# max-andr/joint-cnn-mrf

Measured on AMD Instinct MI355X. Metric: images/sec (720x480, K=9 joints) part-detector+spatial-model fwd, higher is better.
Workload: dtype f32(fp16x2 spectra, fft); 1 GPU; configs[1]: batch=64/GPU synthetic 480x720x3, part detector + spatial model forward + argmax, fp32; batch_per_gpu=64, global_batch=64, micro_batch=64, use_sm=True, collective=all_gather coords int32 [B,2,9]

## Files before the change

### joint-cnn-mrf_amd/csrc/conv_fft.hip

```cpp
#include <cmath>
#include <cstdlib>
#include <map>
#include <mutex>
#include <utility>
#include <vector>

#include "conv_fft_common.h"

namespace jcm {
namespace cfft {

template <int KS, int NP>
__global__ __launch_bounds__(256) void weight_spectra_split_kernel(const float* __restrict__ w, uint4* __restrict__ Ws, int Cin, int Cout, int CoutP, int ntl, int NY, int NX,
                                                                   int round_bf16, float* __restrict__ wscale) {
  __shared__ cf twy[192][KS - 1], twx[KS];
  const int tid = threadIdx.x;
  const int kx = blockIdx.y;
#pragma unroll 1
  for (int k = tid; k < NY * (KS - 1) + KS; k += 256) {
    const bool isy = k < NY * (KS - 1);
    const int ky = k / (KS - 1), a = isy ? k % (KS - 1) + 1 : k - NY * (KS - 1);
    const int num = isy ? (ky * a) % NY : (kx * a) % NX, den = isy ? NY : NX;
    double sn, cs;
    sincospi(-2.0 * (double)num / (double)den, &sn, &cs);
// ... 129 lines not shown
    if (v == n) return off;
    off += v;
  }
  return -1;
}
static bool sizes_of(int H, int W, int ks, Sizes* s, int circ = 0) {
  if (circ) {
    s->NY = H; s->NX = W;
    return (ks == 9 || ks == 5) && H > 8 && W > 8 && tw_offset(H) >= 0 && tw_offset(W) >= 0;
  }
  return (ks == 9 || ks == 5) && H + ks - 1 <= 192 && W + ks - 1 <= 192 && pick(H + 4, &s->NY) && pick(W + 4, &s->NX);
}
static int pad64(int c) { return (c + CB - 1) / CB * CB; }
static bool fft_reg_on() {
  static const bool on = [] { const char* e = std::getenv("JCM_FFT_REG"); return !e || std::atoi(e) != 0; }();
  return on;
}
static int padn(int c, int n) { return (c + n - 1) / n * n; }

int persistent_grid(const void* kernel, int ntiles, int threads, int dyn_lds) {
  static std::mutex mu;
  static std::map<std::pair<const void*, int>, int> cache;
  int dev = 0;
  (void)hipGetDevice(&dev);
  int resident = 0;
  {
    std::lock_guard<std::mutex> lk(mu);
    auto it = cache.find({kernel, dev});
    if (it != cache.end()) resident = it->second;
  }
// ... 76 lines not shown
  p.F = s.NY * p.NXH;
  p.ldy = padn(a.Cout, cgemm_split_ntile(np, a.Cout));
  if (p.ldy < pad64(a.Cout)) p.ldy = pad64(a.Cout);
  p.MT = cgemm_split_mtile(np, a.B, a.Cout);
  const size_t cop = pad64(a.Cout), cmax = (size_t)a.Cin > cop ? a.Cin : cop;
  const size_t bp = (size_t)(a.B + p.MT - 1) / p.MT * p.MT;
  p.t_bytes = (size_t)a.B * p.NXH * a.H * cmax * sizeof(cf);
  p.xs_bytes = (size_t)p.F * bp * a.Cin * 4 * cgemm_split_parts(np);
  p.yf_bytes = (size_t)p.F * a.B * p.ldy * sizeof(cf);
  p.inv_cb = s.NY > 100 ? 32 : 64;
  p.sc_fwd_bytes = (size_t)a.B * a.H * (a.Cin / CB) * sizeof(float);
  p.sc_inv_bytes = (size_t)a.B * p.NXH * (cop / p.inv_cb) * sizeof(float);
  return p;
}
size_t align256(size_t v) { return (v + 255) & ~size_t(255); }
}
size_t conv_fft_workspace_bytes(const ConvArgs& a, int ks, int np) {
  Sizes s;
  if (!sizes_of(a.H, a.W, ks, &s, a.circ)) return 0;
  const Plan3 p = plan_of(a, s, np);
  return align256(p.t_bytes) + align256(p.xs_bytes) + align256(p.yf_bytes) + align256(p.sc_fwd_bytes) + align256(p.sc_inv_bytes);
}
bool conv_fft_fusable(const ConvArgs& a, int ks, int ks_next) {
  Sizes s, n;
  return sizes_of(a.H, a.W, ks, &s) && sizes_of(a.H, a.W, ks_next, &n) && s.NX == n.NX && a.Cout % CB == 0;
}
size_t conv_fft_handover_bytes(const ConvArgs& a, int ks) {
  Sizes s;
  if (!sizes_of(a.H, a.W, ks, &s)) return 0;
  return (size_t)a.B * (s.NX / 2 + 1) * a.H * a.Cout * sizeof(cf);
}
bool conv_fft_win_gather_supported(int win, int Cin) { return fft_reg_on() && cfft_rows_fwd_win_reg_supported(win, Cin); }
bool conv_fft_win_scatter_supported(int win, int Cout) { return fft_reg_on() && win == 32 && Cout % 64 == 0; }
bool conv_fft_pool_fusable(const ConvArgs& a, int ks, int ks_next) {
  Sizes s, n;
  return sizes_of(a.H, a.W, ks, &s) && sizes_of((a.H + 1) / 2, (a.W + 1) / 2, ks_next, &n) && cfft_rows_inv_pool_fwd_supported(s.NX, n.NX, a.Cout);
}
size_t conv_fft_pool_handover_bytes(const ConvArgs& a, int ks_next) {
  Sizes n;
  if (!sizes_of((a.H + 1) / 2, (a.W + 1) / 2, ks_next, &n)) return 0;
  return (size_t)a.B * (n.NX / 2 + 1) * ((a.H + 1) / 2) * a.Cout * sizeof(cf);
}
bool conv_fft_merge_fusable(const ConvArgs& a, int ks, int ks_next, const FftMerge& m, bool h16) {
  Sizes s;
  if (!conv_fft_fusable(a, ks, ks_next) || !sizes_of(a.H, a.W, ks, &s)) return false;
  const bool reg = fft_reg_on() && cfft_rows_inv_merge_fwd_reg_supported(s.NX, a, m, (ks - 1) / 2);
  return h16 ? reg : (reg || cfft_rows_inv_merge_fwd_supported(s.NX, a, m));
}
hipError_t conv_fft_f32(const ConvArgs& a0, int ks, int np, int in_layout, int out_layout, void* work, const void* t_in, void* t_next, const FftMerge* merge,
                        hipEvent_t g0, hipEvent_t g1, hipStream_t st, void* xs, bool xs_ready, const Fp16Scale* scp, const FftNext* nx) {
  Sizes s;
  if (!conv_fft_supported(a0, ks) || !sizes_of(a0.H, a0.W, ks, &s, a0.circ) || (out_layout == 2 && a0.Cout % 8) || (np != 2 && np != 4 && np != 5) || (np == 5 && a0.Cin % 32)) return hipErrorInvalidValue;
  if (a0.circ && (t_in || t_next || merge || in_layout != 0 || out_layout != 0)) return hipErrorInvalidValue;
  if (nx && (nx->pool || nx->merge) && (!t_next || (nx->pool && nx->merge))) return hipErrorInvalidValue;
  Fp16Scale sc;
  if (np >= 4) {
    if (!scp || !scp->tmax || !scp->winv || (t_next && !scp->tmax_next)) return hipErrorInvalidValue;
    sc = *scp;
    sc.hf = (float)a0.H;
    sc.nb = a0.B;
  }
  const bool h16 = sc.t16 && ((t_next && nx && nx->merge && !t_in) || (t_in && !t_next));
  if ((t_in || t_next) && !h16 && (in_layout != 0 || out_layout != 0)) return hipErrorInvalidValue;
  if (t_next && a0.Cout % CB) return hipErrorInvalidValue;
  if (sc.t16 && (np != 5 || in_layout == 0 || out_layout == 0 || xs || ((t_in || t_next) && !h16))) return hipErrorInvalidValue;
// ... 96 lines not shown
```

### joint-cnn-mrf_amd/csrc/conv_fft_common.h

```cpp
#pragma once
#include "fft_lds.h"
#include "kernels.h"

namespace jcm {
namespace cfft {
using namespace fftl;
constexpr int CB = 64, NT = 256;
constexpr int kParMax = 512;

template <int N> struct Plan;
template <> struct Plan<192> { static constexpr int R1 = 8, R2 = 8, R3 = 3; };
template <> struct Plan<128> { static constexpr int R1 = 8, R2 = 4, R3 = 4; };
template <> struct Plan<100> { static constexpr int R1 = 4, R2 = 5, R3 = 5; };
template <> struct Plan<96> { static constexpr int R1 = 8, R2 = 12, R3 = 1; };
template <> struct Plan<72> { static constexpr int R1 = 8, R2 = 3, R3 = 3; };
template <> struct Plan<64> { static constexpr int R1 = 8, R2 = 8, R3 = 1; };
template <> struct Plan<60> { static constexpr int R1 = 4, R2 = 15, R3 = 1; };
template <> struct Plan<50> { static constexpr int R1 = 5, R2 = 10, R3 = 1; };
template <> struct Plan<40> { static constexpr int R1 = 8, R2 = 5, R3 = 1; };
template <> struct Plan<36> { static constexpr int R1 = 4, R2 = 3, R3 = 3; };
template <> struct Plan<32> { static constexpr int R1 = 8, R2 = 4, R3 = 1; };
template <> struct Plan<28> { static constexpr int R1 = 4, R2 = 7, R3 = 1; };
template <> struct Plan<24> { static constexpr int R1 = 8, R2 = 3, R3 = 1; };
template <> struct Plan<20> { static constexpr int R1 = 4, R2 = 5, R3 = 1; };
// ... 230 lines not shown
    default: CALL(192); break;                   \
  }

int persistent_grid(const void* kernel, int ntiles, int threads, int dyn_lds = 0);

void cfft_rows_fwd(int NX, const ConvArgs& a, int layout, cf* T, const cf* tw, float* tmax, hipStream_t st, float* t16 = nullptr);
void cfft_rows_fwd_merge(int NX, const ConvArgs& a, const FftMerge& m, int in_layout, cf* T, const cf* tw, float* tmax, hipStream_t st, float* t16 = nullptr);
hipError_t cfft_cols_fwd(int NY, const ConvArgs& a, int np, const cf* T, void* Xs, const cf* tw, int NXH, int MT, const Fp16Scale& sc, hipStream_t st);
void cfft_cols_inv(int NY, const ConvArgs& a, const cf* Yf, cf* T, const cf* tw, int NXH, int ldy, int pad, hipStream_t st, float* t16 = nullptr, float y16_inv = 0.f);
void cfft_rows_inv(int NX, const ConvArgs& a, int layout, const cf* T, const cf* tw, int pad, float norm, const Fp16Scale& sc, hipStream_t st);
bool cfft_rows_inv_reg(int NX, const ConvArgs& a, int layout, const cf* T, int pad, float norm, const Fp16Scale& sc, hipStream_t st);
bool cfft_rows_inv_fwd_reg(int NX, const ConvArgs& a, const cf* T, cf* Tn, int pad, float norm, const Fp16Scale& sc, hipStream_t st);
bool cfft_rows_fwd_reg(int NX, const ConvArgs& a, int layout, cf* T, float* tmax, hipStream_t st, float* t16);
bool cfft_rows_fwd_win_reg(int NX, const ConvArgs& a, cf* T, float* tmax, hipStream_t st);
bool cfft_rows_fwd_win_reg_supported(int NX, int Cin);
bool cfft_rows_fwd_merge_reg(int NX, const ConvArgs& a, const FftMerge& m, int in_layout, cf* T, float* tmax, hipStream_t st, float* t16);
bool cfft_cols_inv_reg(int NY, const ConvArgs& a, const cf* Yf, cf* T, int NXH, int ldy, int pad, hipStream_t st, float* t16, float y16_inv = 0.f);
void cfft_rows_inv_fwd(int NX, const ConvArgs& a, const cf* T, cf* Tn, const cf* tw, int pad, float norm, const Fp16Scale& sc, hipStream_t st);
bool cfft_rows_inv_pool_fwd(int NXI, int NXO, const ConvArgs& a, const cf* T, cf* Tn, const cf* twi, const cf* two, int pad, float norm, const Fp16Scale& sc, hipStream_t st);
bool cfft_rows_inv_merge_fwd(int NX, const ConvArgs& a, const FftMerge& m, const cf* T, cf* Tn, const cf* tw, int pad, float norm, const Fp16Scale& sc, hipStream_t st);
bool cfft_rows_inv_merge_fwd_reg(int NX, const ConvArgs& a, const FftMerge& m, const cf* T, cf* Tn, int pad, float norm, const Fp16Scale& sc, hipStream_t st, float* t16n = nullptr);
bool cfft_rows_inv_merge_fwd_reg_supported(int NX, const ConvArgs& a, const FftMerge& m, int pad);
bool cfft_rows_inv_pool_fwd_supported(int NXI, int NXO, int Cout);
bool cfft_rows_inv_mfma(int NX, const ConvArgs& a, int layout, const cf* T, int pad, float norm, const Fp16Scale& sc, hipStream_t st);
bool cfft_rows_inv_merge_fwd_supported(int NX, const ConvArgs& a, const FftMerge& m);
}
}
```

### joint-cnn-mrf_amd/csrc/conv_fft_rows_reg.hip

```cpp
#include "conv_fft_common.h"
#include "fft_reg.h"
#include "resize_tf1.h"

namespace jcm {
namespace cfft {
using namespace fftr;

template <int NX, int K1, bool ALL = false, class St>
__device__ __forceinline__ void inv_rows_out2(const cf (&u)[NX / 2], int h, int W, int pad, St&& store) {
  constexpr int M = NX / 2, R1 = RPlan<M>::R1, R2 = RPlan<M>::R2;
  cf o[R2];
  step2_row<M, 1, K1>(u, o);
#pragma unroll
  for (int k2 = 0; k2 < R2; ++k2) {
    const int xo = 2 * (K1 + R1 * k2) + h - pad;
    if (ALL || (xo >= 0 && xo < W)) store(K1 + R1 * k2, xo, o[k2]);
  }
  __builtin_amdgcn_sched_barrier(0);
  if constexpr (K1 + 1 < R1) inv_rows_out2<NX, K1 + 1, ALL>(u, h, W, pad, store);
}
template <int NX, int N>
__device__ __forceinline__ void inv_rows_in2(cf (&u)[NX / 2], const float4& q1, const float4& q2, float sg, bool odd) {
  constexpr int M = NX / 2;
  if constexpr (N == 0) {
// ... 479 lines not shown
  }
  __builtin_amdgcn_sched_barrier(0);
  unsigned raw[M];
  merge_px<NX, W, W3, 0>(raw, r1, v2, v3, odd);
  fwd_rows_finish<NX>(raw, T, h, p, b, y, B, H, C, tmax, t16);
}
bool cfft_rows_fwd_merge_reg(int NX, const ConvArgs& a, const FftMerge& m, int in_layout, cf* T, float* tmax, hipStream_t st, float* t16) {
  if (NX != 96 || in_layout != 1 || !t16 || a.Cin % 64 || a.W != 90 || m.W2 != 45 || m.W3 != 23 || m.H2 < 1 || m.H3 < 1) return false;
  const int nrows = a.B * a.H;
  const size_t threads = a.Cin == 512 ? (size_t)((nrows + 3) / 4) * 8 * 256 : (size_t)nrows * a.Cin;
  hipLaunchKernelGGL((rows_fwd_merge_reg_kernel<96, 90, 23>), dim3((unsigned)((threads + 255) / 256)), dim3(256), 0, st, static_cast<const unsigned*>(a.x), static_cast<const unsigned*>(m.x2), m.H2,
                     static_cast<const unsigned*>(m.x3), m.H3, reinterpret_cast<uint2*>(T), nrows, a.B, a.H, a.Cin, (float)m.H2 / (float)a.H, (float)m.H3 / (float)a.H, tmax, t16);
  return true;
}

template <int NX, int PAD, int I, class Act>
__device__ __forceinline__ void fused_rows_mid(const cf (&x)[NX / 2], cf (&uu)[NX / 2], bool odd, int h, int W, Act&& act) {
  constexpr int M = NX / 2, R1 = RPlan<M>::R1, R2 = RPlan<M>::R2, Q = M / 2;
  constexpr int ma = I + PAD / 2, mb = I + Q + PAD / 2;
  cf a = cf{0.f, 0.f}, bq = cf{0.f, 0.f};
  if constexpr (ma < M) { if (2 * I + h < W) a = act(x[R2 * (ma % R1) + ma / R1]); }
  if constexpr (mb < M) { if (2 * (I + Q) + h < W) bq = act(x[R2 * (mb % R1) + mb / R1]); }
  const cf sm = a + bq, df = a - bq;
  const cf keep = cf{odd ? df.x : sm.x, odd ? df.y : sm.y}, send = cf{odd ? sm.x : df.x, odd ? sm.y : df.y};
  const cf recv = cf{__uint_as_float((unsigned)__builtin_amdgcn_mov_dpp((int)__float_as_uint(send.x), 0xB1, 0xF, 0xF, true)),
                     __uint_as_float((unsigned)__builtin_amdgcn_mov_dpp((int)__float_as_uint(send.y), 0xB1, 0xF, 0xF, true))};
  cf e = cf{odd ? recv.x : keep.x, odd ? recv.y : keep.y}, o = cf{odd ? keep.x : recv.x, odd ? keep.y : recv.y};
  if constexpr (I > 0) {
    const float wr = odd ? Tw<-2 * I, NX>::re : 1.f, wi = odd ? Tw<-2 * I, NX>::im : 0.f;
    e = cf{fmaf(-e.y, wi, e.x * wr), fmaf(e.x, wi, e.y * wr)};
  }
  {
    const float wr = odd ? Tw<-(2 * I + 1), NX>::re : 1.f, wi = odd ? Tw<-(2 * I + 1), NX>::im : 0.f;
    o = cf{fmaf(-o.y, wi, o.x * wr), fmaf(o.x, wi, o.y * wr)};
  }
  uu[2 * I] = e;
  uu[2 * I + 1] = o;
  if constexpr (I + 1 < Q) fused_rows_mid<NX, PAD, I + 1>(x, uu, odd, h, W, act);
}
template <int NX, int PAD>
__global__ __launch_bounds__(256) __attribute__((amdgpu_waves_per_eu(2, 2))) void rows_inv_fwd_reg_kernel(const float4* __restrict__ T, float4* __restrict__ Tn, const float* __restrict__ bias,
                                                                                                  const float* __restrict__ scale, const float* __restrict__ shift, int relu_bn, int nrows,
                                                                                                  int B, int H, int W, int C, float norm0, Fp16Scale sc) {
  constexpr int NXH = NX / 2 + 1, M = NX / 2;
  const int CP = C >> 1;
  const size_t g = (size_t)blockIdx.x * 256 + threadIdx.x;
  const int h = (int)(g & 1), lane = threadIdx.x & 63;
  const int p = (int)((g >> 1) % CP);
  const size_t by = (size_t)(unsigned)__builtin_amdgcn_readfirstlane((int)((g >> 1) / CP));
  if (by >= (size_t)nrows) return;
  const int b = (int)(by / H), y = (int)(by % H), c = 2 * p;
  const bool odd = h != 0;
// ... 287 lines not shown
  else if (layout == 1 && a.Cout % 8 == 0) RR_LAUNCH(1, false);
  else if (layout == 2 && h16 && a.Cout % 8 == 0) RR_LAUNCH(2, true);
  else if (layout == 2 && a.Cout % 8 == 0) RR_LAUNCH(2, false);
  else return false;
#undef RR_LAUNCH
  return true;
}
bool cfft_rows_inv_reg(int NX, const ConvArgs& a, int layout, const cf* T, int pad, float norm, const Fp16Scale& sc, hipStream_t st) {
  if (NX == 96) return launch_rows_inv_reg<96>(a, layout, T, pad, norm, sc, st);
  if (NX == 32 && layout == 0) return launch_rows_inv_reg<32>(a, layout, T, pad, norm, sc, st);
  if (NX == 50) return launch_rows_inv_reg<50>(a, layout, T, pad, norm, sc, st);
  if (NX == 28) return launch_rows_inv_reg<28>(a, layout, T, pad, norm, sc, st);
  return false;
}

}
}
```

### joint-cnn-mrf_amd/csrc/ctx.h

```cpp
#pragma once
#include "../../include/jcm.h"

#include <map>
#include <mutex>
#include <string>
#include <vector>

#include "kernels.h"

namespace jcm {

struct CallOrder;

int fail(int code, const std::string& msg);

#define HIP_TRY(expr)                                                                                   \
  do {                                                                                                  \
    hipError_t e_ = (expr);                                                                             \
    if (e_ != hipSuccess)                                                                               \
      return ::jcm::fail(JCM_ERR_HIP, std::string(#expr) + ": " + hipGetErrorString(e_));               \
  } while (0)
#define JCM_TRY(expr)          \
  do {                         \
    int r_ = (expr);           \
// ... 63 lines not shown
  float* sp_energy = nullptr;
  float* sp_bias = nullptr;
  float* bn_sm_scale = nullptr;
  float* bn_sm_shift = nullptr;
  int* cond = nullptr;
  const float** energy_ptrs = nullptr;
  const float** bias_ptrs = nullptr;
  int* cond0 = nullptr;
  int sm_algo = 3;
  void* fft_t_next = nullptr;
  const void* fft_t_in = nullptr;
  void* fft_xs = nullptr;
  bool fft_xs_ready = false;
  void* sm_scratch = nullptr;
  unsigned sm_epoch = 0;
  int fft_fuse = 3;
  int bf16_hpool = 1;
  int conv_hpool = 0;
  int fft_rows_mfma = 1;
  int fft_next_pool = 0, fft_next_ks = 0;
  const void* fft_win_map = nullptr;
  int fft_win_B = 0, fft_win_H = 0, fft_win_W = 0, fft_win_TY = 0, fft_win_TX = 0;
  bool fft_win_scatter = false;
  bool fft_t_in_16 = false;
  const void* fft_next_merge = nullptr;
  const void* fft_merge = nullptr;
  int conv9_fft = 1;
  int fft_single = 1;
  int fft_win = 1;
  int fft_t16 = 1;
// ... 100 lines not shown
```

### joint-cnn-mrf_amd/csrc/jcm_api.hip

```cpp
#include <cmath>
#include <cstdlib>
#include <cstdio>
#include <cstring>

#include <mutex>
#include <vector>

#include "ctx.h"

using namespace jcm;

namespace {
thread_local std::string g_err;
}

namespace jcm {

const char* const kJointNames[10] = {"lsho", "lelb", "lwri", "rsho", "relb", "rwri", "lhip", "rhip", "nose", "torso"};

int fail(int code, const std::string& msg) {
  g_err = msg;
  return code;
}

// ... 235 lines not shown
    if (hipError_t e = hipMemsetAsync(b.p, 0, (size_t)b.cap * sizeof(float), c->stream); e != hipSuccess) {
      (void)hipFree(b.p);
      return fail(JCM_ERR_HIP, std::string("hipMemsetAsync: ") + hipGetErrorString(e));
    }
    c->fft_blocks.push_back(b);
  }
}
int run_conv_fft(jcm_ctx* c, const ConvLayer* L, const std::string& scope, const void* x, int B, int H, int W, void* out, int in_layout, int out_layout, int circ) {
  ConvArgs a{};
  a.x = x; a.bias = L->bias; a.scale = L->scale; a.shift = L->shift; a.out = out;
  a.B = B; a.H = H; a.W = W; a.Cin = L->cin; a.Cout = L->cout; a.CoutP = L->cout; a.relu_bn = L->has_bn ? 1 : 0;
  a.circ = circ;
  a.rows_mfma = c->fft_rows_mfma;
  const size_t mark = c->arena_off;
  const int np = fft_np(c);
  void* work = arena_alloc<char>(c, conv_fft_workspace_bytes(a, L->ks, np));
  c->arena_off = mark;
  if (c->dry) { c->fft_t_in = nullptr; c->fft_t_next = nullptr; c->fft_merge = nullptr; c->fft_xs = nullptr; c->fft_xs_ready = false; c->fft_tmax_in = nullptr; c->fft_next_pool = 0; c->fft_next_ks = 0; c->fft_next_merge = nullptr; c->fft_t_in_16 = false; c->fft_win_map = nullptr; c->fft_win_scatter = false; return JCM_OK; }
  const std::string key = scope + (circ ? "@win" : "@") + std::to_string(H) + "x" + std::to_string(W);
  if (!c->fft_w.count(key)) {
    static const size_t cap = [] { const char* e = std::getenv("JCM_FFT_CACHE_GB"); return (size_t)(e ? std::atoi(e) : 64) << 30; }();
    const size_t need = conv_fft_weight_bytes(H, W, L->ks, L->cin, L->cout, np, circ);
    size_t held = 0;
    for (auto& kv : c->fft_w) held += kv.second.bytes;
    if (held + need > cap && !c->fft_w.empty()) {
      HIP_TRY(hipStreamSynchronize(c->stream));
      for (auto& kv : c->fft_w) (void)hipFree(kv.second.p);
      c->fft_w.clear();
    }
  }
  jcm_ctx::FftW& fw = c->fft_w[key];
  if (!fw.p) {
    const size_t wb = (conv_fft_weight_bytes(H, W, L->ks, L->cin, L->cout, np, circ) + 255) & ~size_t(255);
    fw.bytes = wb + 256;
    if (hipMalloc(&fw.p, fw.bytes) == hipSuccess) {
      fw.wscale = reinterpret_cast<float*>(static_cast<char*>(fw.p) + wb);
    } else {
      const size_t mb = fw.bytes >> 20;
      c->fft_w.erase(key);
      return fail(JCM_ERR_HIP, "out of device memory for the filter spectra of '" + scope + "' (" + std::to_string(mb) + " MB); jcm_set_option(\"conv9_fft\", 0) selects the direct kernels");
    }
  }
  if (!fw.valid) {
    const float* bound_from = nullptr;
    if (np >= 4 && scope.compare(0, 6, "dgrad:") == 0) {
      auto it = c->fft_w.find(key.substr(6));
      if (it != c->fft_w.end() && it->second.valid && it->second.wscale) bound_from = it->second.wscale;
    }
    HIP_TRY(conv_fft_pack_weights(L->w_raw, fw.p, H, W, L->ks, L->cin, L->cout, np, c->precision == JCM_PRECISION_BF16, c->stream, fw.wscale, circ, bound_from));
    fw.valid = true;
  }
  a.wp = fw.p;
  hipEvent_t e0 = nullptr, e1 = nullptr, g0 = nullptr, g1 = nullptr;
  JCM_TRY(prof_begin(c, &e0, &e1));
  if (c->profile && (pool_get(c, &g0) != JCM_OK || pool_get(c, &g1) != JCM_OK)) { g0 = g1 = nullptr; }
  const void* t_in = c->fft_t_in;
  void* t_next = c->fft_t_next;
  const FftMerge* mg = static_cast<const FftMerge*>(c->fft_merge);
  void* xs = c->fft_xs;
  const bool xs_ready = c->fft_xs_ready;
  FftNext nx;
  nx.pool = c->fft_next_pool; nx.ks_next = c->fft_next_ks; nx.merge = static_cast<const FftMerge*>(c->fft_next_merge);
  c->fft_next_pool = 0; c->fft_next_ks = 0; c->fft_next_merge = nullptr;
  const bool t_in_16 = c->fft_t_in_16;
  c->fft_t_in_16 = false;
  if (c->fft_win_map) {
    a.win_map = c->fft_win_map; a.win_B = c->fft_win_B; a.win_H = c->fft_win_H; a.win_W = c->fft_win_W; a.win_TY = c->fft_win_TY; a.win_TX = c->fft_win_TX;
    c->fft_win_map = nullptr;
  }
  if (c->fft_win_scatter) {
    a.wout_H = c->fft_win_H; a.wout_W = c->fft_win_W; a.wout_TY = c->fft_win_TY; a.wout_TX = c->fft_win_TX;
    c->fft_win_scatter = false;
  }
  Fp16Scale sc;
  if (np >= 4) {
    sc.tmax = c->fft_tmax_in;
    if ((t_in || xs_ready) && !sc.tmax) return fail(JCM_ERR_STATE, "conv_fft '" + scope + "': a handed-over tensor without its scale word");
    if (!sc.tmax) JCM_TRY(fft_new_words(c, B, &sc.tmax));
    if (t_next) JCM_TRY(fft_new_words(c, B, &sc.tmax_next));
    sc.winv = fw.wscale + 1;
    sc.common = c->train ? 1 : 0;
    sc.t16 = (np == 5 && c->fft_t16 && in_layout != 0 && out_layout != 0 && !xs && (!t_in || t_in_16) && (!t_next || (nx.merge && !t_in))) ? 1 : 0;
  }
  c->fft_t_in = nullptr; c->fft_t_next = nullptr; c->fft_merge = nullptr; c->fft_xs = nullptr; c->fft_xs_ready = false;
  c->fft_tmax_in = sc.tmax_next;
  c->fft_last_tmax = sc.tmax;
  const hipError_t e = conv_fft_f32(a, L->ks, np, in_layout, out_layout, work, t_in, t_next, mg, g0, g1, c->stream, xs, xs_ready, np >= 4 ? &sc : nullptr, &nx);
  if (g0 && g1 && e == hipSuccess) c->prof[scope + "/gemm"].emplace_back(g0, g1);
  else { if (g0) c->event_pool.push_back(g0); if (g1) c->event_pool.push_back(g1); }
  prof_end(c, scope, e0, e1, e == hipSuccess);
  if (e != hipSuccess) return fail(JCM_ERR_HIP, std::string("conv_fft_f32: ") + hipGetErrorString(e));
  return JCM_OK;
}
// ... 419 lines not shown
    if ((value != 0) != (h->fft_single != 0)) {
      HIP_TRY(hipStreamSynchronize(h->stream));
      for (auto& kv : h->fft_w) (void)hipFree(kv.second.p);
      h->fft_w.clear();
    }
    h->fft_single = value != 0;
    return JCM_OK;
  }
  if (k == "fft_windows") {
    h->fft_win = value != 0;
    return JCM_OK;
  }
  if (k == "fft_fuse") {
    if (value < 0 || value > 3) return fail(JCM_ERR_ARG, "fft_fuse must be 0..3 (bit 0: pool hand-over, bit 1: merge hand-over)");
    h->fft_fuse = (int)value;
    return JCM_OK;
  }
  if (k == "bf16_hpool") {
    h->bf16_hpool = value != 0;
    return JCM_OK;
  }
  if (k == "fft_rows_mfma") {
    h->fft_rows_mfma = value != 0;
    return JCM_OK;
  }
  if (k == "fft_t16") {
    h->fft_t16 = value != 0;
    return JCM_OK;
  }
  if (k == "sm_chunk") {
// ... 408 lines not shown
```

### joint-cnn-mrf_amd/csrc/kernels.h

```cpp
#pragma once
#include <hip/hip_runtime.h>
#include <stdint.h>

#include <atomic>

namespace jcm {

struct LdsAttr {
  std::atomic<uint64_t> done{0};
  hipError_t ensure(const void* fn, int bytes) {
    int dev = 0;
    hipError_t e = hipGetDevice(&dev);
    if (e != hipSuccess) return e;
    const uint64_t bit = 1ull << (dev & 63);
    if (done.load(std::memory_order_acquire) & bit) return hipSuccess;
    e = hipFuncSetAttribute(fn, hipFuncAttributeMaxDynamicSharedMemorySize, bytes);
    if (e == hipSuccess) done.fetch_or(bit, std::memory_order_release);
    return e;
  }
};

struct ConvArgs {
  const void* x;
  const void* wp;
  const float* bias;
  const float* scale;
  const float* shift;
  void* out;
  int B, H, W, Cin, Cout, CoutP;
  int relu_bn;
  const float* in_scale = nullptr;
  const float* w_scale = nullptr;
  int in_planar = 0, out_planar = 0;
  int circ = 0;
  const void* win_map = nullptr;
  int win_B = 0, win_H = 0, win_W = 0, win_TY = 0, win_TX = 0, win_valid_only = 0;
  int wout_H = 0, wout_W = 0, wout_TY = 0, wout_TX = 0;
  int rows_mfma = 0;
  int hpool = 0;
};
int conv_igemm_bn(int Cout);
hipError_t conv_igemm_f32(const ConvArgs& a, int ks, hipStream_t st);
hipError_t pack_weights_f32(const float* w_hwio, float* wp, int ks, int Cin, int Cout, int CoutP, hipStream_t st);

bool conv_split_supported(int ks, int Cin, int CoutP, int B, int H, int W, int min_wgs);
size_t conv_split_weight_bytes(int ks, int Cin, int CoutP, int ns);
hipError_t pack_weights_split(const float* w_hwio, void* wp, int ks, int Cin, int Cout, int CoutP, int ns, hipStream_t st,
                              const float* w_scale = nullptr);
hipError_t conv_split_f32(const ConvArgs& a, int ks, int ns, hipStream_t st);

hipError_t conv_thin_split16(const ConvArgs& a, hipStream_t st);

// ... 14 lines not shown
  int t16_cb = 64;
};
bool conv_fft_supported(const ConvArgs& a, int ks);
size_t conv_fft_weight_bytes(int H, int W, int ks, int Cin, int Cout, int np, int circ = 0);
hipError_t conv_fft_pack_weights(const float* w_hwio, void* wf, int H, int W, int ks, int Cin, int Cout, int np, bool round_bf16, hipStream_t st,
                                 float* wscale = nullptr, int circ = 0,
                                 const float* bound_from = nullptr);
size_t conv_fft_workspace_bytes(const ConvArgs& a, int ks, int np);
struct FftMerge { const void* x2; int H2, W2; const void* x3; int H3, W3; };
struct FftNext { int pool = 0; int ks_next = 0; const FftMerge* merge = nullptr; };
hipError_t conv_fft_f32(const ConvArgs& a, int ks, int np, int in_layout, int out_layout, void* work, const void* t_in, void* t_next, const FftMerge* merge,
                        hipEvent_t g0, hipEvent_t g1, hipStream_t st, void* xs = nullptr, bool xs_ready = false, const Fp16Scale* sc = nullptr, const FftNext* nx = nullptr);
bool conv_fft_win_gather_supported(int win, int Cin);
bool conv_fft_win_scatter_supported(int win, int Cout);
bool conv_fft_pool_fusable(const ConvArgs& a, int ks, int ks_next);
size_t conv_fft_pool_handover_bytes(const ConvArgs& a, int ks_next);
bool conv_fft_merge_fusable(const ConvArgs& a, int ks, int ks_next, const FftMerge& m, bool h16 = false);
size_t conv_fft_xs_bytes(const ConvArgs& a, int ks, int np);
hipError_t conv_fft_spectra(const ConvArgs& a, int ks, int np, void* work, void* xs, hipStream_t st, float* tmax = nullptr, int common = 0);
bool conv_fft_geometry(int H, int W, int ks, int B, int Cout, int np, int* NY, int* NX, int* MT, int circ = 0);

size_t wgrad_fft_scratch_bytes(int NY, int NX, int Cin, int Cout);
hipError_t wgrad_fft(const void* xs, const void* zs, void* scratch, const float* w, float lmbd, float* dw, int ks, int NY, int NX, int B, int MTx, int MTz, int Cin,
                     int ldz, int Cout, hipStream_t st, int np = 3, const float* tmax_x = nullptr, const float* tmax_z = nullptr, int H = 0);
hipError_t pad_channels_f32(const float* in, int ldi, float* out, int ldo, size_t N, hipStream_t st);
hipError_t window_gather_f32(const float* map, float* win, int B, int H, int W, int C, int WS, int TY, int TX, int valid_only, hipStream_t st);
hipError_t window_scatter_f32(const float* val, float* map, int B, int H, int W, int C, int WS, int TY, int TX, hipStream_t st);
bool conv_fft_fusable(const ConvArgs& a, int ks, int ks_next);
size_t conv_fft_handover_bytes(const ConvArgs& a, int ks);

// ... 147 lines not shown
```

### joint-cnn-mrf_amd/engine.py

```python
import ctypes

import numpy as np
import torch

from . import _lib


def _hm_size(n):
    for _ in range(3):
        n = (n + 1) // 2
    return n


class Engine:

    def __init__(self, device=0, precision='fp32', n_joints=9, stream=None, f32_conv=None, split_min_wgs=None, micro_batch=None, conv9_fft=None, call_order=None, fft_single=None, fft_t16=None, fft_fuse=None):
        if not torch.cuda.is_available():
            raise RuntimeError('joint-cnn-mrf_amd needs an MI355X (gfx950) GPU; torch.cuda.is_available() is False '
                               'and there is no CPU path')
        self._lib = _lib.load()
        self.device = torch.device('cuda', device if isinstance(device, int) else torch.device(device).index or 0)
        self.n_joints = int(n_joints)
        self.precision = precision
        self._stream = stream if stream is not None else torch.cuda.current_stream(self.device)
        h = ctypes.c_void_p()
        _lib.check(self._lib.jcm_create(self.device.index, ctypes.c_void_p(self._stream.cuda_stream), ctypes.byref(h)),
                   'jcm_create')
        self._h = h
        self._finalized = False
        prec = {'fp32': _lib.JCM_PRECISION_F32, 'f32': _lib.JCM_PRECISION_F32, 'bf16': _lib.JCM_PRECISION_BF16}[precision]
        _lib.check(self._lib.jcm_set_option(self._h, b'precision', prec), 'jcm_set_option(precision)')
        _lib.check(self._lib.jcm_set_option(self._h, b'n_joints', self.n_joints), 'jcm_set_option(n_joints)')
        if f32_conv is not None:
            if f32_conv not in ('exact', 'split16'):
                raise ValueError("f32_conv must be 'exact' or 'split16' (the bf16x6 arm 'split' was retired in round 5)")
            _lib.check(self._lib.jcm_set_option(self._h, b'f32_conv', {'exact': 0, 'split16': 2}[f32_conv]), 'jcm_set_option(f32_conv)')
        if micro_batch is not None:
            self.set_micro_batch(micro_batch)
        if conv9_fft is not None:
            self.set_conv9_fft(conv9_fft)
        if fft_single is not None:
            self.set_option('fft_single', int(bool(fft_single)))
        if fft_t16 is not None:
            self.set_option('fft_t16', int(bool(fft_t16)))
        if fft_fuse is not None:
            self.set_option('fft_fuse', int(fft_fuse))
        if call_order is not None:
            self.set_option('call_order', int(bool(call_order)))
        if split_min_wgs is not None:
            _lib.check(self._lib.jcm_set_option(self._h, b'split_min_wgs', int(split_min_wgs)), 'jcm_set_option(split_min_wgs)')

    def close(self):
        if getattr(self, '_h', None) is not None and self._h.value:
            self._lib.jcm_destroy(self._h)
            self._h = ctypes.c_void_p()

    def __del__(self):
        try:
            self.close()
        except Exception:
            pass
# ... 292 lines not shown
```

Measured before the change: 7014 images/sec.

## Split 5x5 FFT convolution into four overlap-save tiles with fused pool hand-over

Adds a tiled FFT convolution path for the 5x5 layer feeding a pooled 5x5 layer: each image is cut into four quadrants with halos, transformed at a smaller FFT size (64x96), convolved per tile, and the inverse row pass stitches the two column tiles, pools and produces the next layer's forward row spectra. The smaller transform size is meant to cut FFT padding overhead and spectrum memory for the full-resolution layer. It adds new row kernels, per-tile scale words and separate weight spectra keyed by the tile size. The cost is halo recomputation and more complex indexing, and the path is restricted to width 180.

```diff
diff --git a/joint-cnn-mrf_amd/csrc/conv_fft.hip b/joint-cnn-mrf_amd/csrc/conv_fft.hip
--- a/joint-cnn-mrf_amd/csrc/conv_fft.hip
+++ b/joint-cnn-mrf_amd/csrc/conv_fft.hip
@@ -167,6 +167,10 @@
 static int pad64(int c) { return (c + CB - 1) / CB * CB; }
 static bool fft_reg_on() {
   static const bool on = [] { const char* e = std::getenv("JCM_FFT_REG"); return !e || std::atoi(e) != 0; }();
+  return on;
+}
+static bool fft_tiles_on() {
+  static const bool on = [] { const char* e = std::getenv("JCM_FFT_TILES"); return !e || std::atoi(e) != 0; }();
   return on;
 }
 static int padn(int c, int n) { return (c + n - 1) / n * n; }
@@ -273,11 +277,17 @@
   return p;
 }
 size_t align256(size_t v) { return (v + 255) & ~size_t(255); }
+ConvArgs tile_view(const ConvArgs& a, const Sizes& s) {
+  ConvArgs t = a;
+  t.B = 4 * a.B; t.H = s.NY; t.W = a.W / 2;
+  t.tiles = 0;
+  return t;
+}
 }
 size_t conv_fft_workspace_bytes(const ConvArgs& a, int ks, int np) {
   Sizes s;
-  if (!sizes_of(a.H, a.W, ks, &s, a.circ)) return 0;
-  const Plan3 p = plan_of(a, s, np);
+  if (!(a.tiles ? sizes_of(a.H / 2, a.W / 2, ks, &s) : sizes_of(a.H, a.W, ks, &s, a.circ))) return 0;
+  const Plan3 p = a.tiles ? plan_of(tile_view(a, s), s, np) : plan_of(a, s, np);
   return align256(p.t_bytes) + align256(p.xs_bytes) + align256(p.yf_bytes) + align256(p.sc_fwd_bytes) + align256(p.sc_inv_bytes);
 }
 bool conv_fft_fusable(const ConvArgs& a, int ks, int ks_next) {
@@ -300,14 +310,53 @@
   if (!sizes_of((a.H + 1) / 2, (a.W + 1) / 2, ks_next, &n)) return 0;
   return (size_t)a.B * (n.NX / 2 + 1) * ((a.H + 1) / 2) * a.Cout * sizeof(cf);
 }
+bool conv_fft_tiles_supported(const ConvArgs& a, int ks, int ks_next) {
+  Sizes s;
+  return fft_reg_on() && fft_tiles_on() && ks == 5 && ks_next == 5 && !a.circ && !a.win_map && a.B >= 1 && conv_fft_pool_fusable(a, ks, ks_next) &&
+         a.H % 4 == 0 && a.W % 4 == 0 && sizes_of(a.H / 2, a.W / 2, ks, &s) && cfft_tiles_supported(s.NY, s.NX, a);
+}
 bool conv_fft_merge_fusable(const ConvArgs& a, int ks, int ks_next, const FftMerge& m, bool h16) {
   Sizes s;
   if (!conv_fft_fusable(a, ks, ks_next) || !sizes_of(a.H, a.W, ks, &s)) return false;
   const bool reg = fft_reg_on() && cfft_rows_inv_merge_fwd_reg_supported(s.NX, a, m, (ks - 1) / 2);
   return h16 ? reg : (reg || cfft_rows_inv_merge_fwd_supported(s.NX, a, m));
 }
+static hipError_t conv_fft_tiles_f32(const ConvArgs& a0, int ks, int np, int in_layout, void* work, const void* t_in, void* t_next, const FftMerge* merge,
+                                     hipEvent_t g0, hipEvent_t g1, hipStream_t st, void* xs, bool xs_ready, const Fp16Scale* scp, const FftNext* nx) {
+  Sizes s;
+  if (np != 4 || in_layout != 0 || t_in || merge || xs || xs_ready || !t_next || !nx || !nx->pool || nx->merge || !scp || !scp->tmax || !scp->winv || !scp->tmax_next ||
+      !conv_fft_tiles_supported(a0, ks, nx->ks_next) || !sizes_of(a0.H / 2, a0.W / 2, ks, &s))
+    return hipErrorInvalidValue;
+  ConvArgs a = a0;
+  a.CoutP = pad64(a.Cout);
+  const ConvArgs at = tile_view(a, s);
+  const Plan3 p = plan_of(at, s, np);
+  Fp16Scale sc = *scp;
+  sc.hf = (float)s.NY;
+  sc.nb = at.B;
+  char* wk = static_cast<char*>(work);
+  cf* T = reinterpret_cast<cf*>(wk);
+  void* Xs = wk + align256(p.t_bytes);
+  cf* Yf = reinterpret_cast<cf*>(wk + align256(p.t_bytes) + align256(p.xs_bytes));
+  int dev = 0;
+  if (hipError_t e = hipGetDevice(&dev); e != hipSuccess) return e;
+  const cf* twb = twiddle_table(dev);
+  if (!twb) return hipErrorOutOfMemory;
+  if (!cfft_rows_fwd_tile_reg(s.NY, s.NX, a, T, sc.tmax, st)) return hipErrorInvalidValue;
+  if (hipError_t ce = cfft_cols_fwd(s.NY, at, np, T, Xs, twb + tw_offset(s.NY), p.NXH, p.MT, sc, st); ce != hipSuccess) return ce;
+  if (hipError_t e = hipGetLastError(); e != hipSuccess) return e;
+  if (g0 && hipEventRecord(g0, st) != hipSuccess) return hipErrorUnknown;
+  if (hipError_t e = cgemm_split(Xs, a.wp, Yf, np, p.F, at.B, a.Cin, a.Cout, p.ldy, st, 0.f); e != hipSuccess) return e;
+  if (g1 && hipEventRecord(g1, st) != hipSuccess) return hipErrorUnknown;
+  ConvArgs ai = at;
+  ai.H = a.H / 2;
+  if (!cfft_cols_inv_reg(s.NY, ai, Yf, T, p.NXH, p.ldy, (ks - 1) / 2, st, nullptr, 0.f)) return hipErrorInvalidValue;
+  if (!cfft_rows_inv_pool_tile_reg(s.NY, s.NX, a, T, static_cast<cf*>(t_next), 1.0f / (float)(s.NY * s.NX), sc, st)) return hipErrorInvalidValue;
+  return hipGetLastError();
+}
 hipError_t conv_fft_f32(const ConvArgs& a0, int ks, int np, int in_layout, int out_layout, void* work, const void* t_in, void* t_next, const FftMerge* merge,
                         hipEvent_t g0, hipEvent_t g1, hipStream_t st, void* xs, bool xs_ready, const Fp16Scale* scp, const FftNext* nx) {
+  if (a0.tiles) return conv_fft_tiles_f32(a0, ks, np, in_layout, work, t_in, t_next, merge, g0, g1, st, xs, xs_ready, scp, nx);
   Sizes s;
   if (!conv_fft_supported(a0, ks) || !sizes_of(a0.H, a0.W, ks, &s, a0.circ) || (out_layout == 2 && a0.Cout % 8) || (np != 2 && np != 4 && np != 5) || (np == 5 && a0.Cin % 32)) return hipErrorInvalidValue;
   if (a0.circ && (t_in || t_next || merge || in_layout != 0 || out_layout != 0)) return hipErrorInvalidValue;
diff --git a/joint-cnn-mrf_amd/csrc/conv_fft_common.h b/joint-cnn-mrf_amd/csrc/conv_fft_common.h
--- a/joint-cnn-mrf_amd/csrc/conv_fft_common.h
+++ b/joint-cnn-mrf_amd/csrc/conv_fft_common.h
@@ -268,6 +268,9 @@
 bool cfft_rows_fwd_reg(int NX, const ConvArgs& a, int layout, cf* T, float* tmax, hipStream_t st, float* t16);
 bool cfft_rows_fwd_win_reg(int NX, const ConvArgs& a, cf* T, float* tmax, hipStream_t st);
 bool cfft_rows_fwd_win_reg_supported(int NX, int Cin);
+bool cfft_tiles_supported(int NY, int NX, const ConvArgs& a);
+bool cfft_rows_fwd_tile_reg(int NY, int NX, const ConvArgs& a, cf* T, float* tmax, hipStream_t st);
+bool cfft_rows_inv_pool_tile_reg(int NY, int NX, const ConvArgs& a, const cf* T, cf* Tn, float norm, const Fp16Scale& sc, hipStream_t st);
 bool cfft_rows_fwd_merge_reg(int NX, const ConvArgs& a, const FftMerge& m, int in_layout, cf* T, float* tmax, hipStream_t st, float* t16);
 bool cfft_cols_inv_reg(int NY, const ConvArgs& a, const cf* Yf, cf* T, int NXH, int ldy, int pad, hipStream_t st, float* t16, float y16_inv = 0.f);
 void cfft_rows_inv_fwd(int NX, const ConvArgs& a, const cf* T, cf* Tn, const cf* tw, int pad, float norm, const Fp16Scale& sc, hipStream_t st);
diff --git a/joint-cnn-mrf_amd/csrc/conv_fft_rows_reg.hip b/joint-cnn-mrf_amd/csrc/conv_fft_rows_reg.hip
--- a/joint-cnn-mrf_amd/csrc/conv_fft_rows_reg.hip
+++ b/joint-cnn-mrf_amd/csrc/conv_fft_rows_reg.hip
@@ -1,3 +1,5 @@
+#include <type_traits>
+
 #include "conv_fft_common.h"
 #include "fft_reg.h"
 #include "resize_tf1.h"
@@ -517,13 +519,8 @@
   return true;
 }
 
-template <int NX, int PAD, int I, class Act>
-__device__ __forceinline__ void fused_rows_mid(const cf (&x)[NX / 2], cf (&uu)[NX / 2], bool odd, int h, int W, Act&& act) {
-  constexpr int M = NX / 2, R1 = RPlan<M>::R1, R2 = RPlan<M>::R2, Q = M / 2;
-  constexpr int ma = I + PAD / 2, mb = I + Q + PAD / 2;
-  cf a = cf{0.f, 0.f}, bq = cf{0.f, 0.f};
-  if constexpr (ma < M) { if (2 * I + h < W) a = act(x[R2 * (ma % R1) + ma / R1]); }
-  if constexpr (mb < M) { if (2 * (I + Q) + h < W) bq = act(x[R2 * (mb % R1) + mb / R1]); }
+template <int NX, int I>
+__device__ __forceinline__ void fwd_rows_mid_pair(const cf a, const cf bq, cf (&uu)[NX / 2], bool odd) {
   const cf sm = a + bq, df = a - bq;
   const cf keep = cf{odd ? df.x : sm.x, odd ? df.y : sm.y}, send = cf{odd ? sm.x : df.x, odd ? sm.y : df.y};
   const cf recv = cf{__uint_as_float((unsigned)__builtin_amdgcn_mov_dpp((int)__float_as_uint(send.x), 0xB1, 0xF, 0xF, true)),
@@ -539,6 +536,15 @@
   }
   uu[2 * I] = e;
   uu[2 * I + 1] = o;
+}
+template <int NX, int PAD, int I, class Act>
+__device__ __forceinline__ void fused_rows_mid(const cf (&x)[NX / 2], cf (&uu)[NX / 2], bool odd, int h, int W, Act&& act) {
+  constexpr int M = NX / 2, R1 = RPlan<M>::R1, R2 = RPlan<M>::R2, Q = M / 2;
+  constexpr int ma = I + PAD / 2, mb = I + Q + PAD / 2;
+  cf a = cf{0.f, 0.f}, bq = cf{0.f, 0.f};
+  if constexpr (ma < M) { if (2 * I + h < W) a = act(x[R2 * (ma % R1) + ma / R1]); }
+  if constexpr (mb < M) { if (2 * (I + Q) + h < W) bq = act(x[R2 * (mb % R1) + mb / R1]); }
+  fwd_rows_mid_pair<NX, I>(a, bq, uu, odd);
   if constexpr (I + 1 < Q) fused_rows_mid<NX, PAD, I + 1>(x, uu, odd, h, W, act);
 }
 template <int NX, int PAD>
@@ -856,5 +862,199 @@
   return false;
 }
 
-}
-}
+
+template <int NX, int J>
+__device__ __forceinline__ void fwd_rows_in2_f32(cf (&u)[NX / 2], const cf (&raw)[NX / 2], float sg, bool odd) {
+  constexpr int M = NX / 2;
+  const cf a = raw[J], o = cf{__uint_as_float(pair_word(__float_as_uint(a.x), odd)), __uint_as_float(pair_word(__float_as_uint(a.y), odd))};
+  cf v = cf{fmaf(sg, a.x, o.x), fmaf(sg, a.y, o.y)};
+  if constexpr (J > 0) {
+    const float wr = odd ? Tw<-J, NX>::re : 1.f, wi = odd ? Tw<-J, NX>::im : 0.f;
+    v = cf{fmaf(-v.y, wi, v.x * wr), fmaf(v.x, wi, v.y * wr)};
+  }
+  u[J] = v;
+  if constexpr (J + 1 < M) fwd_rows_in2_f32<NX, J + 1>(u, raw, sg, odd);
+}
+template <int NX>
+__global__ __launch_bounds__(256) __attribute__((amdgpu_waves_per_eu(3, 3))) void rows_fwd_tile_reg_kernel(const float* __restrict__ map, float4* __restrict__ T, int nrows, int NY,
+                                                                                                   int Hm, int Wm, int Ht, int Wt, int C, float* __restrict__ tmax) {
+  constexpr int M = NX / 2;
+  const int CP = C >> 1;
+  int h, p;
+  size_t by;
+  pair_coords(CP, h, p, by);
+  if (by >= (size_t)nrows) return;
+  const int bt = (int)(by / NY), t = (int)(by % NY);
+  const int tx = bt & 1, ty = (bt >> 1) & 1, b = bt >> 2;
+  const int ym = t < Ht + 2 ? ty * Ht + t : (t >= NY - 2 ? ty * Ht + t - NY : -1);
+  const bool row_in = ym >= 0 && ym < Hm;
+  const auto d = __builtin_amdgcn_make_buffer_rsrc(const_cast<float*>(map) + ((size_t)b * Hm + (row_in ? ym : 0)) * Wm * C, 0, row_in ? Wm * C * 4 : 0, 0x00020000);
+  cf raw[M];
+  typedef float f2 __attribute__((ext_vector_type(2)));
+#pragma unroll
+  for (int j = 0; j < M; ++j) {
+    const int n = h * M + j;
+    const int xm = n < Wt + 2 ? tx * Wt + n : (n >= NX - 2 ? tx * Wt + n - NX : -1);
+    const int off = xm >= 0 && xm < Wm ? xm * C * 4 : Wm * C * 4;
+    raw[j] = __builtin_bit_cast(cf, __builtin_amdgcn_raw_buffer_load_b64(d, p * 8 + off, 0, 0));
+  }
+  const bool odd = h != 0;
+  cf u[M];
+  fwd_rows_in2_f32<NX, 0>(u, raw, odd ? -1.f : 1.f, odd);
+  step1<M, -1>(u);
+  step2_inplace<M, -1, 0>(u);
+  const int cblk = p >> 5, v = p & 31, B4 = nrows / NY;
+  float4* dst = T + ((((size_t)cblk * 4 + (v >> 3)) * B4 + bt) * NY + t) * 8 + (v & 7);
+  const size_t kstride = (size_t)(C >> 4) * B4 * NY * 8;
+  float m = 0.f;
+  fwd_rows_visit<NX, 0>(u, odd, [&](int mi, const float4& o) __attribute__((always_inline)) {
+    const int k = 2 * mi + h;
+    if (k <= M) {
+      dst[(size_t)k * kstride] = o;
+      m = fmaxf(fmaxf(m, fmaxf(fabsf(o.x), fabsf(o.y))), fmaxf(fabsf(o.z), fabsf(o.w)));
+    }
+  });
+  if (tmax) {
+#pragma unroll
+    for (int o = 32; o > 0; o >>= 1) m = fmaxf(m, __shfl_xor(m, o));
+    if ((threadIdx.x & 63) == 0 && m > 0.f) atomicMax(reinterpret_cast<unsigned*>(tmax + bt), __float_as_uint(m));
+  }
+}
+
+template <int NX, int TX, int I, int WT, class Act>
+__device__ __forceinline__ void pool_tile_px(const cf x, cf (&zp)[NX / 2], bool odd, bool first, Act&& act) {
+  const cf v = act(x);
+  const cf w = cf{__uint_as_float((unsigned)__builtin_amdgcn_mov_dpp((int)__float_as_uint(v.x), 0xB1, 0xF, 0xF, true)),
+                  __uint_as_float((unsigned)__builtin_amdgcn_mov_dpp((int)__float_as_uint(v.y), 0xB1, 0xF, 0xF, true))};
+  const cf pm = cf{fmaxf(v.x, w.x), fmaxf(v.y, w.y)};
+  constexpr int q = TX * (WT / 2) + I;
+  if (((q & 1) != 0) == odd) zp[q >> 1] = first ? pm : cf{fmaxf(zp[q >> 1].x, pm.x), fmaxf(zp[q >> 1].y, pm.y)};
+}
+template <int NX, int TX, int K1, int K2, int WT, class Act>
+__device__ __forceinline__ void pool_tile_outs(const cf (&o)[RPlan<NX / 2>::R2], cf (&zp)[NX / 2], bool odd, bool first, Act&& act) {
+  constexpr int I = K1 + RPlan<NX / 2>::R1 * K2 - 1;
+  if constexpr (I >= 0 && I < WT / 2) pool_tile_px<NX, TX, I, WT>(o[K2], zp, odd, first, act);
+  if constexpr (K2 + 1 < RPlan<NX / 2>::R2) pool_tile_outs<NX, TX, K1, K2 + 1, WT>(o, zp, odd, first, act);
+}
+template <int NX, int TX, int K1, int WT, class Act>
+__device__ __forceinline__ void pool_tile_row(const cf (&u)[NX / 2], cf (&zp)[NX / 2], bool odd, bool first, Act&& act) {
+  constexpr int M = NX / 2;
+  cf o[RPlan<M>::R2];
+  step2_row<M, 1, K1>(u, o);
+  pool_tile_outs<NX, TX, K1, 0, WT>(o, zp, odd, first, act);
+  __builtin_amdgcn_sched_barrier(0);
+  if constexpr (K1 + 1 < RPlan<M>::R1) pool_tile_row<NX, TX, K1 + 1, WT>(u, zp, odd, first, act);
+}
+template <int NX, int I>
+__device__ __forceinline__ void pool_rows_mid(const cf (&zp)[NX / 2], cf (&uu)[NX / 2], bool odd) {
+  fwd_rows_mid_pair<NX, I>(zp[I], zp[I + NX / 4], uu, odd);
+  if constexpr (I + 1 < NX / 4) pool_rows_mid<NX, I + 1>(zp, uu, odd);
+}
+template <int NX, int WT>
+__global__ __launch_bounds__(256) __attribute__((amdgpu_waves_per_eu(2, 2))) void rows_inv_pool_tile_reg_kernel(const float4* __restrict__ T, float4* __restrict__ Tn, const float* __restrict__ bias,
+                                                                                                        const float* __restrict__ scale, const float* __restrict__ shift, int relu_bn,
+                                                                                                        int nrows, int B, int Ht, int C, float norm0, Fp16Scale sc) {
+  constexpr int NXH = NX / 2 + 1, M = NX / 2;
+  static_assert(WT % 2 == 0 && WT + 4 <= NX, "even tile width with its halo inside the transform");
+  const int CP = C >> 1;
+  const size_t g = (size_t)blockIdx.x * 256 + threadIdx.x;
+  const int h = (int)(g & 1), lane = threadIdx.x & 63;
+  const int p = (int)((g >> 1) % CP);
+  const size_t by = (size_t)(unsigned)__builtin_amdgcn_readfirstlane((int)((g >> 1) / CP));
+  if (by >= (size_t)nrows) return;
+  const int b = (int)(by / Ht), r = (int)(by % Ht), c = 2 * p;
+  constexpr int KS = (WT / 2 - 1) / 2;
+  __shared__ cf stash[4][KS][64];
+  const int ty = (2 * r) / Ht, yt = 2 * r - ty * Ht;
+  const bool odd = h != 0;
+  const float b0v = bias[c], b1v = bias[c + 1];
+  float s0 = 1.f, s1 = 1.f, h0 = 0.f, h1 = 0.f;
+  if (relu_bn) { s0 = scale[c]; h0 = shift[c]; s1 = scale[c + 1]; h1 = shift[c + 1]; }
+  float tcommon = 0.f;
+  if (sc.tmax && sc.common) {
+    for (int i = lane; i < sc.nb; i += 64) tcommon = fmaxf(tcommon, sc.tmax[i]);
+#pragma unroll
+    for (int o = 32; o > 0; o >>= 1) tcommon = fmaxf(tcommon, __shfl_xor(tcommon, o));
+  }
+  cf zp[M];
+#pragma unroll
+  for (int k = 0; k < M; ++k) zp[k] = cf{0.f, 0.f};
+  auto tile = [&](auto txc) __attribute__((always_inline)) {
+    constexpr int tx = decltype(txc)::value;
+    const int bt = (b * 2 + ty) * 2 + tx;
+    const float norm = sc.tmax ? norm0 * sc.winv[0] * fp16_unscale(sc.common ? tcommon : sc.tmax[bt], sc.hf) : norm0;
+    auto act = [&](cf z) __attribute__((always_inline)) {
+      float v0 = fmaf(z.x, norm, b0v), v1 = fmaf(z.y, norm, b1v);
+      if (relu_bn) { v0 = fmaf(fmaxf(v0, 0.f), s0, h0); v1 = fmaf(fmaxf(v1, 0.f), s1, h1); }
+      return cf{v0, v1};
+    };
+#pragma unroll
+    for (int rr = 0; rr < 2; ++rr) {
+      __builtin_amdgcn_sched_barrier(0);
+      cf u[M];
+      const auto d = __builtin_amdgcn_make_buffer_rsrc(const_cast<float4*>(T) + (((size_t)bt * Ht + yt + rr) * NXH * C) / 2, 0, NXH * C * 8, 0x00020000);
+      const int vo = p * 16, ko = CP * 16;
+      auto load = [&](int k) __attribute__((always_inline)) {
+        typedef float f4 __attribute__((ext_vector_type(4)));
+        const f4 q = __builtin_bit_cast(f4, __builtin_amdgcn_raw_buffer_load_b128(d, vo, k * ko, 0));
+        return make_float4(q[0], q[1], q[2], q[3]);
+      };
+      int hr = h;
+      asm volatile("" : "+v"(hr));
+      const bool odd_r = hr != 0;
+      inv_rows_load2<NX, false, 0>(u, odd_r ? -1.f : 1.f, odd_r, load);
+      step1<M, 1>(u);
+      pool_tile_row<NX, tx, 0, WT>(u, zp, odd, rr == 0, act);
+    }
+  };
+  cf(*const slice)[64] = stash[threadIdx.x >> 6];
+  tile(std::integral_constant<int, 0>{});
+#pragma unroll
+  for (int k = 0; k < KS; ++k) slice[k][lane] = zp[k];
+  tile(std::integral_constant<int, 1>{});
+#pragma unroll
+  for (int k = 0; k < KS; ++k) zp[k] = slice[k][lane];
+  cf uu[M];
+  pool_rows_mid<NX, 0>(zp, uu, odd);
+  step1<M, -1>(uu);
+  step2_inplace<M, -1, 0>(uu);
+  const int cblk = p >> 5, v = p & 31;
+  float4* dst = Tn + ((((size_t)cblk * 4 + (v >> 3)) * B + b) * Ht + r) * 8 + (v & 7);
+  const size_t kstride = (size_t)(C >> 4) * B * Ht * 8;
+  float m = 0.f;
+  fwd_rows_visit<NX, 0>(uu, odd, [&](int mi, const float4& o) __attribute__((always_inline)) {
+    const int k = 2 * mi + h;
+    if (k <= M) {
+      dst[(size_t)k * kstride] = o;
+      m = fmaxf(fmaxf(m, fmaxf(fabsf(o.x), fabsf(o.y))), fmaxf(fabsf(o.z), fabsf(o.w)));
+    }
+  });
+  if (sc.tmax_next) {
+#pragma unroll
+    for (int o = 32; o > 0; o >>= 1) m = fmaxf(m, __shfl_xor(m, o));
+    if (lane == 0 && m > 0.f) atomicMax(reinterpret_cast<unsigned*>(sc.tmax_next + b), __float_as_uint(m));
+  }
+}
+bool cfft_tiles_supported(int NY, int NX, const ConvArgs& a) {
+  return NX == 96 && NY == 64 && a.W == 180 && a.H % 4 == 0 && a.H / 2 + 4 <= NY && a.Cin % 64 == 0 && a.Cout % 64 == 0 &&
+         (size_t)a.W * a.Cin * 4 < (size_t)1 << 31;
+}
+bool cfft_rows_fwd_tile_reg(int NY, int NX, const ConvArgs& a, cf* T, float* tmax, hipStream_t st) {
+  if (!cfft_tiles_supported(NY, NX, a)) return false;
+  const int nrows = 4 * a.B * NY;
+  const size_t threads = (size_t)nrows * a.Cin;
+  hipLaunchKernelGGL(rows_fwd_tile_reg_kernel<96>, dim3((unsigned)((threads + 255) / 256)), dim3(256), 0, st, static_cast<const float*>(a.x), reinterpret_cast<float4*>(T), nrows, NY,
+                     a.H, a.W, a.H / 2, a.W / 2, a.Cin, tmax);
+  return true;
+}
+bool cfft_rows_inv_pool_tile_reg(int NY, int NX, const ConvArgs& a, const cf* T, cf* Tn, float norm, const Fp16Scale& sc, hipStream_t st) {
+  if (!cfft_tiles_supported(NY, NX, a)) return false;
+  const int Ht = a.H / 2, nrows = a.B * Ht;
+  const size_t threads = (size_t)nrows * a.Cout;
+  hipLaunchKernelGGL((rows_inv_pool_tile_reg_kernel<96, 90>), dim3((unsigned)((threads + 255) / 256)), dim3(256), 0, st, reinterpret_cast<const float4*>(T), reinterpret_cast<float4*>(Tn),
+                     a.bias, a.scale, a.shift, a.relu_bn, nrows, a.B, Ht, a.Cout, norm, sc);
+  return true;
+}
+
+}
+}
diff --git a/joint-cnn-mrf_amd/csrc/ctx.h b/joint-cnn-mrf_amd/csrc/ctx.h
--- a/joint-cnn-mrf_amd/csrc/ctx.h
+++ b/joint-cnn-mrf_amd/csrc/ctx.h
@@ -101,6 +101,7 @@
   bool fft_xs_ready = false;
   void* sm_scratch = nullptr;
   unsigned sm_epoch = 0;
+  int fft_tiles = 1;
   int fft_fuse = 3;
   int bf16_hpool = 1;
   int conv_hpool = 0;
diff --git a/joint-cnn-mrf_amd/csrc/jcm_api.hip b/joint-cnn-mrf_amd/csrc/jcm_api.hip
--- a/joint-cnn-mrf_amd/csrc/jcm_api.hip
+++ b/joint-cnn-mrf_amd/csrc/jcm_api.hip
@@ -273,13 +273,16 @@
   a.rows_mfma = c->fft_rows_mfma;
   const size_t mark = c->arena_off;
   const int np = fft_np(c);
+  a.tiles = c->fft_tiles && c->fft_next_pool && !c->fft_t_in && !c->fft_xs && !c->fft_merge && !c->fft_win_map && !circ && in_layout == 0 &&
+            np == 4 && conv_fft_tiles_supported(a, L->ks, c->fft_next_ks) ? 1 : 0;
+  const int wH = a.tiles ? H / 2 : H, wW = a.tiles ? W / 2 : W;
   void* work = arena_alloc<char>(c, conv_fft_workspace_bytes(a, L->ks, np));
   c->arena_off = mark;
   if (c->dry) { c->fft_t_in = nullptr; c->fft_t_next = nullptr; c->fft_merge = nullptr; c->fft_xs = nullptr; c->fft_xs_ready = false; c->fft_tmax_in = nullptr; c->fft_next_pool = 0; c->fft_next_ks = 0; c->fft_next_merge = nullptr; c->fft_t_in_16 = false; c->fft_win_map = nullptr; c->fft_win_scatter = false; return JCM_OK; }
-  const std::string key = scope + (circ ? "@win" : "@") + std::to_string(H) + "x" + std::to_string(W);
+  const std::string key = scope + (circ ? "@win" : "@") + std::to_string(wH) + "x" + std::to_string(wW);
   if (!c->fft_w.count(key)) {
     static const size_t cap = [] { const char* e = std::getenv("JCM_FFT_CACHE_GB"); return (size_t)(e ? std::atoi(e) : 64) << 30; }();
-    const size_t need = conv_fft_weight_bytes(H, W, L->ks, L->cin, L->cout, np, circ);
+    const size_t need = conv_fft_weight_bytes(wH, wW, L->ks, L->cin, L->cout, np, circ);
     size_t held = 0;
     for (auto& kv : c->fft_w) held += kv.second.bytes;
     if (held + need > cap && !c->fft_w.empty()) {
@@ -290,7 +293,7 @@
   }
   jcm_ctx::FftW& fw = c->fft_w[key];
   if (!fw.p) {
-    const size_t wb = (conv_fft_weight_bytes(H, W, L->ks, L->cin, L->cout, np, circ) + 255) & ~size_t(255);
+    const size_t wb = (conv_fft_weight_bytes(wH, wW, L->ks, L->cin, L->cout, np, circ) + 255) & ~size_t(255);
     fw.bytes = wb + 256;
     if (hipMalloc(&fw.p, fw.bytes) == hipSuccess) {
       fw.wscale = reinterpret_cast<float*>(static_cast<char*>(fw.p) + wb);
@@ -306,7 +309,7 @@
       auto it = c->fft_w.find(key.substr(6));
       if (it != c->fft_w.end() && it->second.valid && it->second.wscale) bound_from = it->second.wscale;
     }
-    HIP_TRY(conv_fft_pack_weights(L->w_raw, fw.p, H, W, L->ks, L->cin, L->cout, np, c->precision == JCM_PRECISION_BF16, c->stream, fw.wscale, circ, bound_from));
+    HIP_TRY(conv_fft_pack_weights(L->w_raw, fw.p, wH, wW, L->ks, L->cin, L->cout, np, c->precision == JCM_PRECISION_BF16, c->stream, fw.wscale, circ, bound_from));
     fw.valid = true;
   }
   a.wp = fw.p;
@@ -335,7 +338,7 @@
   if (np >= 4) {
     sc.tmax = c->fft_tmax_in;
     if ((t_in || xs_ready) && !sc.tmax) return fail(JCM_ERR_STATE, "conv_fft '" + scope + "': a handed-over tensor without its scale word");
-    if (!sc.tmax) JCM_TRY(fft_new_words(c, B, &sc.tmax));
+    if (!sc.tmax) JCM_TRY(fft_new_words(c, a.tiles ? 4 * B : B, &sc.tmax));
     if (t_next) JCM_TRY(fft_new_words(c, B, &sc.tmax_next));
     sc.winv = fw.wscale + 1;
     sc.common = c->train ? 1 : 0;
@@ -785,6 +788,10 @@
   if (k == "fft_fuse") {
     if (value < 0 || value > 3) return fail(JCM_ERR_ARG, "fft_fuse must be 0..3 (bit 0: pool hand-over, bit 1: merge hand-over)");
     h->fft_fuse = (int)value;
+    return JCM_OK;
+  }
+  if (k == "fft_tiles") {
+    h->fft_tiles = value != 0;
     return JCM_OK;
   }
   if (k == "bf16_hpool") {
diff --git a/joint-cnn-mrf_amd/csrc/kernels.h b/joint-cnn-mrf_amd/csrc/kernels.h
--- a/joint-cnn-mrf_amd/csrc/kernels.h
+++ b/joint-cnn-mrf_amd/csrc/kernels.h
@@ -36,6 +36,7 @@
   const void* win_map = nullptr;
   int win_B = 0, win_H = 0, win_W = 0, win_TY = 0, win_TX = 0, win_valid_only = 0;
   int wout_H = 0, wout_W = 0, wout_TY = 0, wout_TX = 0;
+  int tiles = 0;
   int rows_mfma = 0;
   int hpool = 0;
 };
@@ -80,6 +81,7 @@
 bool conv_fft_win_gather_supported(int win, int Cin);
 bool conv_fft_win_scatter_supported(int win, int Cout);
 bool conv_fft_pool_fusable(const ConvArgs& a, int ks, int ks_next);
+bool conv_fft_tiles_supported(const ConvArgs& a, int ks, int ks_next);
 size_t conv_fft_pool_handover_bytes(const ConvArgs& a, int ks_next);
 bool conv_fft_merge_fusable(const ConvArgs& a, int ks, int ks_next, const FftMerge& m, bool h16 = false);
 size_t conv_fft_xs_bytes(const ConvArgs& a, int ks, int np);
diff --git a/joint-cnn-mrf_amd/engine.py b/joint-cnn-mrf_amd/engine.py
--- a/joint-cnn-mrf_amd/engine.py
+++ b/joint-cnn-mrf_amd/engine.py
@@ -14,7 +14,7 @@
 
 class Engine:
 
-    def __init__(self, device=0, precision='fp32', n_joints=9, stream=None, f32_conv=None, split_min_wgs=None, micro_batch=None, conv9_fft=None, call_order=None, fft_single=None, fft_t16=None, fft_fuse=None):
+    def __init__(self, device=0, precision='fp32', n_joints=9, stream=None, f32_conv=None, split_min_wgs=None, micro_batch=None, conv9_fft=None, call_order=None, fft_single=None, fft_t16=None, fft_fuse=None, fft_tiles=None):
         if not torch.cuda.is_available():
             raise RuntimeError('joint-cnn-mrf_amd needs an MI355X (gfx950) GPU; torch.cuda.is_available() is False '
                                'and there is no CPU path')
@@ -45,6 +45,8 @@
             self.set_option('fft_t16', int(bool(fft_t16)))
         if fft_fuse is not None:
             self.set_option('fft_fuse', int(fft_fuse))
+        if fft_tiles is not None:
+            self.set_option('fft_tiles', int(bool(fft_tiles)))
         if call_order is not None:
             self.set_option('call_order', int(bool(call_order)))
         if split_min_wgs is not None:
```

Result: faster. 7216 images/sec, median of 6 (+2.9%).
